# shanjiayao/PTT

Hardware: AMD Instinct MI355X
Metric: tracklet frames/sec (hot path: PointNet++ SA stack + Point-Track-Transformer blocks) (higher is better)
Workload: dtype f32

## Files before the change

include/ptt_hip.h:

```cpp
#ifndef PTT_HIP_H
#define PTT_HIP_H

#include <stddef.h>
#include <stdint.h>

#ifdef __cplusplus
extern "C" {
#endif

#define PTT_ABI_VERSION 30

enum {
    PTT_OK = 0,
    PTT_EINVAL = -1,
    PTT_EUNSUPPORTED = -2,
    PTT_ELAUNCH = -3,
    PTT_EWORKSPACE = -4
};

typedef void* ptt_stream_t;

int ptt_version(void);
const char* ptt_error_name(int code);
const char* ptt_last_error_string(void);

// ... 6 lines not shown
                 int B, int N, int C, int npoint, int32_t* idx_out, ptt_stream_t stream);

int ptt_gather_f32(const float* feat, const int32_t* idx, int B, int C, int N, int M,
                   float* out, ptt_stream_t stream);
int ptt_gather_grad_f32(const float* grad_out, const int32_t* idx, int B, int C, int N,
                        int M, float* grad_feat, ptt_stream_t stream);

int ptt_select_centres_f32(const float* xyz, const int32_t* idx, int B, int N, int M, float* new_xyz,
                           int64_t* idx64_out, ptt_stream_t stream);

int ptt_ball_query_f32(const float* new_xyz, const float* xyz, int B, int M, int N,
                       float radius, int nsample, int32_t* idx_out, ptt_stream_t stream);

int ptt_centres_ball_query_f32(const float* xyz, const int32_t* sel, int B, int N, int M, float radius, int nsample,
                               float* new_xyz, int64_t* idx64_out, int32_t* idx_out, ptt_stream_t stream);

int ptt_group_f32(const float* feat, const int32_t* idx, int B, int C, int N, int M,
                  int ns, float* out, ptt_stream_t stream);
int ptt_group_grad_f32(const float* grad_out, const int32_t* idx, int B, int C, int N,
                       int M, int ns, float* grad_feat, ptt_stream_t stream);

size_t ptt_scatter_add_det_workspace(int B, int N, int E);
int ptt_scatter_add_det_f32(const float* src, const int32_t* idx, int B, int C, int N, int E, float* out,
                            void* workspace, size_t workspace_bytes, ptt_stream_t stream);

int ptt_knn_f32(const float* xyz, int B, int N, int k, int32_t* idx_out,
                ptt_stream_t stream);
int ptt_knn_rel_f32(const float* xyz, int B, int N, int k, int32_t* idx_out, float* rel_out,
                    ptt_stream_t stream);

// ... 66 lines not shown
    int64_t feat_sb, feat_sc, feat_sn;
    float* out;
    int64_t out_sb, out_sc, out_sm;
    int B, N, M, nsample, C;
    float radius;
    int use_xyz;
    int normalize_xyz;
    int n_layers;
    ptt_sa_layer layers[PTT_SA_MAX_LAYERS];
    const float* l0_point_term;
    const float* l0_xyz_weight;
    int l0_channels;
    int l0_relu;
    void* compact_ws;
    size_t compact_ws_bytes;
} ptt_sa_desc;

int ptt_sa_fused_fwd_f32(const ptt_sa_desc* d, ptt_stream_t stream);
size_t ptt_sa_compact_workspace(int B, int M);

typedef struct ptt_xcorr_desc {
    const float* cos_t;
    const float* P;
    const float* w_sim;
    const float* scale0;
    const float* shift0;
    float* out;
    int64_t out_sb, out_sc, out_sn;
    float* sim_out;
    int B, Ns, Nt, C0;
// ... 369 lines not shown
```

ptt_amd/_lib.py:

```python
import ctypes
import os
import re
from ctypes import Structure, c_char_p, c_double, c_float, c_int, c_int32, c_int64, c_longlong, c_size_t, c_uint32, c_void_p

from .build import HEADER as HEADER_PATH, LIB as LIB_PATH


def _strip_comments(text):
    return re.sub(r"/\*.*?\*/|//[^\n]*", " ", text, flags=re.S)


def parse_defines(text):
    return {n: int(v) for n, v in re.findall(r"^[ \t]*#[ \t]*define[ \t]+(PTT_\w+)[ \t]+(-?\d+)[ \t]*$", _strip_comments(text), re.M)}


CTYPES = {"int": c_int, "int32_t": c_int32, "uint32_t": c_uint32, "int64_t": c_int64, "long long": c_longlong, "size_t": c_size_t,
          "float": c_float, "double": c_double, "ptt_stream_t": c_void_p}


def _ctype(decl, name, is_return=False):
    words = decl.replace("*", " * ").split()
    if not is_return and len(words) > 1 and words[-1] != "*":
        words.pop()
    if "*" in words:
# ... 135 lines not shown


class SaLayer(Structure):
    _fields_ = [("Wpacked", c_void_p), ("scale", c_void_p), ("shift", c_void_p),
                ("Cin", c_int), ("Cout", c_int), ("relu", c_int)]


class SaDesc(Structure):
    _fields_ = [("xyz", c_void_p), ("new_xyz", c_void_p), ("idx", c_void_p), ("feat", c_void_p),
                ("feat_sb", c_int64), ("feat_sc", c_int64), ("feat_sn", c_int64),
                ("out", c_void_p), ("out_sb", c_int64), ("out_sc", c_int64), ("out_sm", c_int64),
                ("B", c_int), ("N", c_int), ("M", c_int), ("nsample", c_int), ("C", c_int),
                ("radius", c_float), ("use_xyz", c_int), ("normalize_xyz", c_int), ("n_layers", c_int),
                ("layers", SaLayer * PTT_SA_MAX_LAYERS),
                ("l0_point_term", c_void_p), ("l0_xyz_weight", c_void_p), ("l0_channels", c_int), ("l0_relu", c_int),
                ("compact_ws", c_void_p), ("compact_ws_bytes", c_size_t)]


class XcorrDesc(Structure):
    _fields_ = [("cos_t", c_void_p), ("P", c_void_p), ("w_sim", c_void_p), ("scale0", c_void_p), ("shift0", c_void_p),
                ("out", c_void_p), ("out_sb", c_int64), ("out_sc", c_int64), ("out_sn", c_int64),
                ("sim_out", c_void_p),
                ("B", c_int), ("Ns", c_int), ("Nt", c_int), ("C0", c_int),
                ("n_layers", c_int), ("layers", SaLayer * PTT_SA_MAX_LAYERS),
                ("split", c_int32), ("out_sh", c_int64), ("search_feat", c_void_p), ("templ_feat", c_void_p),
                ("s_sb", c_int64), ("s_sn", c_int64), ("t_sb", c_int64), ("t_sn", c_int64), ("C", c_int), ("eps", c_float)]


class AttnDesc(Structure):
    _fields_ = [("xyz", c_void_p), ("rel", c_void_p), ("knn", c_void_p), ("qkv", c_void_p),
                ("Wd1p", c_void_p), ("Wd2p", c_void_p), ("bd2", c_void_p),
# ... 36 lines not shown
```

ptt_amd/csrc/common.h:

```cpp
#pragma once
#include <hip/hip_runtime.h>
#include <stdint.h>
#include <stdio.h>
#include "../../include/ptt_hip.h"

namespace ptt {

char* last_error_buf();
int fail(int code, const char* fmt, ...);
int check_launch(const char* what);

static inline hipStream_t as_stream(ptt_stream_t s) { return reinterpret_cast<hipStream_t>(s); }

struct DevSwitches {
    int linear_rt = 1, linear_ct = 1;
    int linear_small = 1;
    int sa_gather1 = 0;
    int sa_stagger = 0;
    int sa_wave = 1;
    int sa_rt = 2;
    int sa_lds = 1;
    int sa_stream = 1;
    int sa_chunk = 2;
    int pair_stagger = 0;
// ... 2 lines not shown
    int fps_plain = 0;
    int ball_cpw = 0;
    int fps_t = 0;
    int ffps_stream = 0;
    int group_grad_global = 0;
    long long* stamps = nullptr;
};
const DevSwitches& dev_switches();

int set_lds_limit(const void* fn, int bytes);

bool wgrad_stream_ok(int R, int Cout, int Cin, int ldz, int ldx);
int wgrad_stream_rows(int R);
int launch_wgrad_stream(const float* dZ, int ldz, const float* X, int ldx, int R, int Cout, int Cin, int rows, float* partial,
                        const float* x_scale, const float* x_shift, hipStream_t s);

template <int CTRL, int ROW_MASK>
__device__ __forceinline__ int dpp_i32(int v) {
    return __builtin_amdgcn_update_dpp(v, v, CTRL, ROW_MASK, 0xF, false);
}
template <int CTRL, int ROW_MASK>
__device__ __forceinline__ float dpp_f32(float v) {
    return __builtin_bit_cast(float, dpp_i32<CTRL, ROW_MASK>(__builtin_bit_cast(int, v)));
}

__device__ __forceinline__ float wave_max_f32(float v) {
    v = fmaxf(v, dpp_f32<0xB1, 0xF>(v));
    v = fmaxf(v, dpp_f32<0x4E, 0xF>(v));
    v = fmaxf(v, dpp_f32<0x141, 0xF>(v));
    v = fmaxf(v, dpp_f32<0x140, 0xF>(v));
// ... 38 lines not shown
```

ptt_amd/csrc/mfma_ops.hip:

```cpp
#include <math.h>
#include <stdlib.h>
#include <string.h>
#include "common.h"
#include "mfma_common.h"

#ifndef PTT_PAIR_PF
#define PTT_PAIR_PF 1
#endif
#ifndef PTT_GATHER_BATCH
#define PTT_GATHER_BATCH 16
#endif
#ifndef PTT_SA_WAVES
#define PTT_SA_WAVES 2
#endif

namespace ptt {

#ifdef PTT_DEV
#define PTT_STAMP(i) do { if (p.dbg && threadIdx.x == 0 && blockIdx.x < 4096) p.dbg[blockIdx.x * 8 + (i)] = __builtin_readcyclecounter(); } while (0)
#else
#define PTT_STAMP(i) do { } while (0)
#endif

__device__ __forceinline__ void stagger_second_slot(int first_wave_blocks, int quanta) {
// ... 1237 lines not shown
                    if (2 * rt < ncentres) {
                        const int c = centre0 + 2 * rt; const int b = c / p.M, mm = c - b * p.M;
                        p.out[b * p.osb + col * p.osc + mm * p.osm] = m0;
                    }
                    if (2 * rt + 1 < ncentres) {
                        const int c = centre0 + 2 * rt + 1; const int b = c / p.M, mm = c - b * p.M;
                        p.out[b * p.osb + col * p.osc + mm * p.osm] = m1;
                    }
                }
            }
        }
    }
    __builtin_amdgcn_wave_barrier();
}

constexpr int SAC_HDR = 16;
struct SacTable {
    int32_t* ws; int T;
    __host__ __device__ int32_t* ndist() const { return ws + SAC_HDR; }
    __host__ __device__ int32_t* list(int k) const { return ws + SAC_HDR + (size_t)(1 + k) * T; }
    __host__ __device__ int32_t* rows(int k) const { return ws + SAC_HDR + 5 * (size_t)T + (size_t)((4 << k) - 4) * T; }
    static size_t words(size_t T) { return SAC_HDR + 65 * T; }
};
constexpr int SAC_PASSES = 4;

__global__ __launch_bounds__(64) void sa_compact_zero_kernel(int32_t* ws) {
    if (threadIdx.x < 4) ws[threadIdx.x] = 0;
}

template <bool XYZ>
__global__ __launch_bounds__(256) void sa_compact_kernel(const float* __restrict__ xyz, const int32_t* __restrict__ idx, int N, int M,
                                                         SacTable tab) {
    __shared__ int s_cnt[4], s_base[4], s_cls[32], s_pos[32], s_nd[32];
    __shared__ int s_row[32][32];
    const int t = threadIdx.x, lane = t & 63, half = lane >> 5, s = lane & 31, w = t >> 6;
    const int g0 = blockIdx.x * 32, T = tab.T;
    if (t < 4) s_cnt[t] = 0;
    __syncthreads();
// ... 814 lines not shown
    p.dbg = dev_switches().stamps;
    p.cws = nullptr;
    const int total_centres = d->B * d->M;
    hipStream_t s = as_stream(stream);
    int rc;
    if (d->C == 0 && d->use_xyz && !hoist && d->nsample == 32 && d->n_layers == 3 && p.L[0].Cout == 64 && p.L[1].Cout == 64 &&
        p.L[2].Cout == 128 && !p.L[0].scale && !p.L[1].scale && !p.L[2].scale && p.L[0].relu && p.L[1].relu &&
        dev_switches().sa_lds) {
        const int waves = 256 * PTT_SAL_WAVES * PTT_SAL_WGS;
        p.chunk = (total_centres + waves - 1) / waves;
        if (dev_switches().sa_lds_chunk > 0 && p.chunk > dev_switches().sa_lds_chunk) p.chunk = dev_switches().sa_lds_chunk;
        const int nw = total_centres * 3 <= 256 * PTT_SAL_WAVES ? 4 : PTT_SAL_WAVES;
        int wgs = (total_centres + p.chunk * nw - 1) / (p.chunk * nw);
        const int lds = (4096 + 8192 + PTT_SAL_WAVES * 640) * (int)sizeof(float);
        if (d->compact_ws) {
            if (d->compact_ws_bytes < ptt_sa_compact_workspace(d->B, d->M) || (reinterpret_cast<uintptr_t>(d->compact_ws) & 15))
                return fail(PTT_EWORKSPACE, "ptt_sa_fused_fwd_f32: compact_ws needs %zu bytes, 16-byte aligned (got %zu)",
                            ptt_sa_compact_workspace(d->B, d->M), d->compact_ws_bytes);
            p.cws = static_cast<int32_t*>(d->compact_ws);
            hipLaunchKernelGGL(sa_compact_zero_kernel, dim3(1), dim3(64), 0, s, p.cws);
            if ((rc = check_launch("sa_compact_zero_kernel"))) return rc;
            hipLaunchKernelGGL(sa_compact_kernel<true>, dim3((total_centres + 31) / 32), dim3(256), 0, s, d->xyz, d->idx, d->N, d->M,
                               SacTable{p.cws, total_centres});
            if ((rc = check_launch("sa_compact_kernel"))) return rc;
            if (wgs > 256 * PTT_SAL_WGS) wgs = 256 * PTT_SAL_WGS;
            if ((rc = set_lds_limit(reinterpret_cast<const void*>(sa_lds_kernel<true>), lds))) return rc;
            hipLaunchKernelGGL(sa_lds_kernel<true>, dim3(wgs), dim3(64 * nw), lds, s, p);
            return check_launch("sa_lds_kernel");
        }
        if ((rc = set_lds_limit(reinterpret_cast<const void*>(sa_lds_kernel<false>), lds))) return rc;
// ... 21 lines not shown
        }
        return check_launch("sa_wave_kernel");
    }
    if (p.hoist == 2 && d->nsample == 32 && d->n_layers == 2 && p.L[0].Cin == 128 && p.L[0].Cout == 128 &&
        p.L[1].Cout == 256 && !p.L[0].scale && !p.L[1].scale && p.L[0].relu && dev_switches().sa_stream) {
        p.tiles = (total_centres + 1) / 2;
        int wgs = p.tiles < 512 ? p.tiles : 512;
        p.chunk = (p.tiles + wgs - 1) / wgs;
        if (dev_switches().sa_chunk > 0 && p.chunk > dev_switches().sa_chunk) p.chunk = dev_switches().sa_chunk;
        wgs = (p.tiles + p.chunk - 1) / p.chunk;
        if (d->compact_ws) {
            if (d->compact_ws_bytes < ptt_sa_compact_workspace(d->B, d->M) || (reinterpret_cast<uintptr_t>(d->compact_ws) & 15))
                return fail(PTT_EWORKSPACE, "ptt_sa_fused_fwd_f32: compact_ws needs %zu bytes, 16-byte aligned (got %zu)",
                            ptt_sa_compact_workspace(d->B, d->M), d->compact_ws_bytes);
            p.cws = static_cast<int32_t*>(d->compact_ws);
            hipLaunchKernelGGL(sa_compact_zero_kernel, dim3(1), dim3(64), 0, s, p.cws);
            if ((rc = check_launch("sa_compact_zero_kernel"))) return rc;
            hipLaunchKernelGGL(sa_compact_kernel<false>, dim3((total_centres + 31) / 32), dim3(256), 0, s, d->xyz, d->idx, d->N, d->M,
                               SacTable{p.cws, total_centres});
            if ((rc = check_launch("sa_compact_kernel"))) return rc;
            const int lds = (2 * SAS_TILE + 64 * 4 + 64) * (int)sizeof(float);
            if ((rc = set_lds_limit(reinterpret_cast<const void*>(sa_stream_compact_kernel), lds))) return rc;
            hipLaunchKernelGGL(sa_stream_compact_kernel, dim3(p.tiles < 512 ? p.tiles : 512), dim3(256), lds, s, p);
            return check_launch("sa_stream_compact_kernel");
        }
        const int lds = (2 * SAS_TILE + 4 * 16 * 4) * (int)sizeof(float);
        if ((rc = set_lds_limit(reinterpret_cast<const void*>(sa_stream_kernel<32>), lds))) return rc;
        hipLaunchKernelGGL((sa_stream_kernel<32>), dim3(wgs), dim3(256), lds, s, p);
        return check_launch("sa_stream_kernel");
    }
    int RT = dev_switches().sa_rt;
    if (d->nsample == 64) RT = 2;
    const int lds = 32 * RT * p.ldk * (int)sizeof(float);
    if (lds > 160 * 1024) return fail(PTT_EUNSUPPORTED, "ptt_sa_fused_fwd_f32: %d B of LDS per workgroup", lds);
    const int cpw = 32 * RT / d->nsample;
// ... 126 lines not shown
```

ptt_amd/csrc/point_ops.hip:

```cpp
#pragma clang fp contract(off)

#include <limits.h>
#include <stdlib.h>
#include "common.h"

namespace ptt {

__device__ __forceinline__ float sqdist3(float ax, float ay, float az, float bx, float by, float bz) {
    const float dx = ax - bx, dy = ay - by, dz = az - bz;
    return (dx * dx + dy * dy) + dz * dz;
}

__device__ __forceinline__ float knn_dist(float ax, float ay, float az, float bx, float by, float bz) {
    const float d = sqdist3(ax, ay, az, bx, by, bz);
    return d < __builtin_inff() ? d : 3.402823466e+38f;
}

__device__ __forceinline__ float lane_bcast(float v, int src_lane) {
    return __builtin_bit_cast(float, __builtin_amdgcn_readlane(__builtin_bit_cast(int, v), src_lane));
}

typedef float fps_f2 __attribute__((ext_vector_type(2)));


// ... 258 lines not shown
    float cx[CPW], cy[CPW], cz[CPW];
    const int nc = min(CPW, BM - centre);
#pragma unroll
    for (int c = 0; c < CPW; ++c) {
        const int cc = centre + (c < nc ? c : 0);
        const int n = sel ? sel[cc] : cc - b * M;
        cx[c] = pts[3 * n + 0]; cy[c] = pts[3 * n + 1]; cz[c] = pts[3 * n + 2];
        if (lane == 0 && c < nc) {
            new_xyz[(size_t)cc * 3 + 0] = cx[c]; new_xyz[(size_t)cc * 3 + 1] = cy[c]; new_xyz[(size_t)cc * 3 + 2] = cz[c];
            if (idx64) idx64[cc] = n;
        }
    }
    ball_sweep<CPW>(pts, N, r2, ns, cx, cy, cz, nc, idx_out + (size_t)centre * ns, lane);
}

__global__ void gather_kernel(const float* __restrict__ feat, const int32_t* __restrict__ idx, int C, int N, int M,
                              float* __restrict__ out, size_t total) {
    for (size_t e = (size_t)blockIdx.x * blockDim.x + threadIdx.x; e < total; e += (size_t)gridDim.x * blockDim.x) {
        const int j = (int)(e % M);
        const size_t bc = e / M;
        const int b = (int)(bc / C);
        out[e] = feat[bc * N + idx[(size_t)b * M + j]];
    }
}
__global__ void gather_grad_kernel(const float* __restrict__ go, const int32_t* __restrict__ idx, int C, int N, int M,
                                   float* __restrict__ gf, size_t total) {
    for (size_t e = (size_t)blockIdx.x * blockDim.x + threadIdx.x; e < total; e += (size_t)gridDim.x * blockDim.x) {
        const int j = (int)(e % M);
        const size_t bc = e / M;
        const int b = (int)(bc / C);
// ... 1021 lines not shown
    if (!xyz || !new_xyz || !idx_out) return fail(PTT_EINVAL, "ptt_centres_ball_query_f32: null pointer");
    const int BM = B * M;
    const int cpw = ball_cpw(BM, M);
    if (cpw == 8)
        hipLaunchKernelGGL((centres_ball_query_kernel<8>), dim3((BM / 8 + 3) / 4), dim3(256), 0, as_stream(stream), xyz, sel, BM,
                           M, N, radius * radius, nsample, new_xyz, reinterpret_cast<long long*>(idx64_out), idx_out);
    else if (cpw == 4)
        hipLaunchKernelGGL((centres_ball_query_kernel<4>), dim3((BM / 4 + 3) / 4), dim3(256), 0, as_stream(stream), xyz, sel, BM,
                           M, N, radius * radius, nsample, new_xyz, reinterpret_cast<long long*>(idx64_out), idx_out);
    else
        hipLaunchKernelGGL((centres_ball_query_kernel<1>), dim3((BM + 3) / 4), dim3(256), 0, as_stream(stream), xyz, sel, BM, M,
                           N, radius * radius, nsample, new_xyz, reinterpret_cast<long long*>(idx64_out), idx_out);
    return check_launch("centres_ball_query_kernel");
}


extern "C" size_t ptt_ball_query_grid_workspace(int B, int N) {
    if (B <= 0 || N <= 0) return 0;
    return (size_t)B * grid_slice_ints(N) * sizeof(int32_t);
}

static int ball_query_grid_launch(const char* who, const float* xyz, const float* centres, const int32_t* sel, int sel_mode, int B, int N, int M,
                                  float radius, int nsample, float* new_xyz, int64_t* idx64, int32_t* idx_out, void* ws, size_t ws_bytes,
                                  ptt_stream_t stream) {
    if (B < 0 || M < 0 || N <= 0 || nsample <= 0) return fail(PTT_EINVAL, "%s: B=%d M=%d N=%d nsample=%d", who, B, M, N, nsample);
    if (B == 0 || M == 0) return PTT_OK;
    if (N > 131072) return fail(PTT_EUNSUPPORTED, "%s: N=%d (the hit bitmap of a wave lives in LDS: at most 131072 points)", who, N);
    if (!ws || ws_bytes < ptt_ball_query_grid_workspace(B, N) || (reinterpret_cast<uintptr_t>(ws) & 15))
        return fail(PTT_EWORKSPACE, "%s: %zu bytes of 16-byte aligned workspace needed", who, ptt_ball_query_grid_workspace(B, N));
    hipStream_t s = as_stream(stream);
// ... 161 lines not shown
```

ptt_amd/models/backbones_3d/pointnet2/pointnet2_modules.py:

```python
import os
from typing import List

import torch
import torch.nn as nn
import torch.nn.functional as F

from .... import ops, train_ops
from ....param_cache import (DropsCachesOnModeChange, FoldedLayer, ParamCache, conv_bn_tensors, fold_conv_bn,
                             index_table)
from . import pointnet2_utils
from . import pytorch_utils as pt_utils

STREAM_COMPACT_MIN_BALLS = 2048
STREAM_COMPACT_MAX_POINTS = 1024


class PointnetSAModuleVotes(DropsCachesOnModeChange, nn.Module):
    def __init__(self, *, mlp: List[int], radius: float = None, nsample: int = None, bn: bool = True,
                 use_xyz: bool = True, normalize_xyz: bool = False, sample_uniformly: bool = False,
                 sample_method='fps'):
        super().__init__()
        self.radius = radius
        self.nsample = nsample
        self.mlp_module = None
# ... 57 lines not shown
            scale, shift = fold_conv_bn(unit)
            scale0 = scale if li == 0 else scale0
            wq = w if scale is None else w * scale.view(-1, 1, 1, 1)
            layers.append(FoldedLayer(ops.pack_weight(wq, rot), None, shift, cin, cout, hasattr(unit, 'activation')))
        hoist = None
        w0 = self.mlp_module[0].conv.weight
        if (self.use_xyz and len(layers) >= 2 and w0.shape[1] > 3 and layers[0].cout <= 256
                and os.environ.get('PTT_SA_HOIST', '1') != '0'):
            w2 = w0.reshape(w0.shape[0], w0.shape[1]).float()
            wx = w2[:, 0:3] if scale0 is None else w2[:, 0:3] * scale0[:, None]
            wf = w2[:, 3:] if scale0 is None else w2[:, 3:] * scale0[:, None]
            hoist = (ops.pack_weight(wf.contiguous()), wx.t().contiguous(), layers[0].cout, layers[0].relu)
        return layers, hoist

    def forward(self, xyz: torch.Tensor, features: torch.Tensor, npoint: int, inds: torch.Tensor = None, pre=None,
                compact: bool = False):
        self.centres_knn = None
        if self._fusable(xyz, features):
            return self._forward_fused(xyz, features, npoint, inds, pre, compact)
        return self._forward_train(xyz, features, npoint, inds)

    def _forward_fused(self, xyz, features, npoint, inds, pre, compact):
        if (pre is None and inds is None and self.sample_method == 'fps' and xyz.shape[1] <= 256 and npoint <= 128
                and xyz.shape[0] * npoint * self.nsample <= ops.ONE_FRAME_MAX_SA_ROWS and self.centres_knn_k <= npoint):
            xyz = xyz.contiguous()
            inds, inds64, new_xyz, idx, self.centres_knn = ops.fps_ball_knn(xyz, npoint, self.radius, self.nsample, self.centres_knn_k)
            pre = (new_xyz, idx, inds64)
        prefix = inds is None and self.sample_method in ('rs', 'sequence')
        if pre is not None:
            pass
        elif prefix:
            inds64 = index_table(xyz.size(0), npoint, xyz.device, torch.int64)
        elif inds is None:
            inds = self._sample(xyz, features, npoint)
        else:
            assert inds.shape[1] == npoint
            inds = inds.to(torch.int32)

        xyz = xyz.contiguous()
        if pre is not None:
            new_xyz, idx, inds64 = pre
        elif prefix:
            new_xyz, _, idx = ops.centres_ball_query(xyz, None, npoint, self.radius, self.nsample)
        else:
            new_xyz, inds64, idx = ops.centres_ball_query(xyz, inds.contiguous(), npoint, self.radius, self.nsample)
        layers, hoist = self._fused_params(xyz.device)
        if hoist is not None and features is not None:
            wf_packed, wx, c0, relu0 = hoist
            rows = features.transpose(1, 2)
            uniform = rows.stride(2) == 1 and rows.stride(0) == rows.shape[1] * rows.stride(1)
            term = ops.linear(rows if uniform else rows.contiguous(), wf_packed, c0, None, layers[0].shift, relu=False)
            B, M, ns = xyz.shape[0], npoint, self.nsample
            if (B * M * ns <= ops.ONE_FRAME_MAX_SA_ROWS and ns in (16, 32) and len(layers) == 3 and c0 % 4 == 0 and c0 >= 192):
                L1, L2 = layers[1], layers[2]
                h = torch.empty((B * M * ns, L1.cout), dtype=torch.float32, device=xyz.device)
                ops.row_jobs([pt_utils.layer_job(L1, prologue=3, x=term, idx=idx, xyz=xyz, centres=new_xyz, wx=wx,
                                                 radius=self.radius, ns=ns, M=M, N=xyz.shape[1], normalize_xyz=self.normalize_xyz,
                                                 pro_relu=relu0, out=h)])
                pooled = torch.empty((B, M, L2.cout), dtype=torch.float32, device=xyz.device)
                ops.row_jobs([pt_utils.layer_job(L2, x=h, epilogue=2, ns=ns, M=M, out=pooled)])
                return new_xyz, pooled.transpose(1, 2), inds64
            new_features = ops.sa_fused_forward(xyz, new_xyz, idx, None, layers[1:], self.radius, True,
                                                self.normalize_xyz, point_major_out=True, l0=(term, wx, relu0),
                                                compact=(bool(compact) and B * M >= STREAM_COMPACT_MIN_BALLS
                                                         and xyz.shape[1] <= STREAM_COMPACT_MAX_POINTS))
        else:
            new_features = ops.sa_fused_forward(xyz, new_xyz, idx, features, layers, self.radius,
                                                self.use_xyz, self.normalize_xyz, point_major_out=True,
                                                compact=features is None)
        return new_xyz, new_features, inds64

    def _forward_train(self, xyz, features, npoint, inds):
        if inds is None:
            inds = self._sample(xyz, features, npoint)
        else:
            assert inds.shape[1] == npoint
            inds = inds.to(torch.int32)
        hoist = (self.use_xyz and not self.sample_uniformly and self.nsample * npoint <= 16384
                 and train_ops.usable(self.mlp_module, xyz if features is None else features)
                 and self.mlp_module[0].conv.weight.shape[0] % 4 == 0)
# ... 17 lines not shown
```

ptt_amd/models/backbones_3d/pointnet2_backbone.py:

```python
from typing import List

import torch
import torch.nn as nn

from ... import graph_policy, ops, train_ops
from ...param_cache import ParamCache, index_table
from .pointnet2 import pointnet2_modules


class PointNet2BackboneLight(nn.Module):
    def __init__(self, model_cfg, input_channels, **kwargs):
        super().__init__()
        self.model_cfg = model_cfg
        input_channels -= 3
        self.num_points_each_layer = []
        self.SA_modules = nn.ModuleList()
        sa = self.model_cfg.SA_CONFIG
        for k in range(len(sa.RADIUS)):
            mlps = list(sa.MLPS[k])
            if k == 0:
                mlps[0] = input_channels
            self.SA_modules.append(pointnet2_modules.PointnetSAModuleVotes(
                radius=sa.RADIUS[k], nsample=sa.NSAMPLE[k], mlp=mlps,
                use_xyz=sa.get('USE_XYZ', True), normalize_xyz=sa.get('NORMALIZE_XYZ', True),
                sample_method=sa.SAMPLE_METHOD[k]))
        self.cov_final = nn.Conv1d(256, 256, kernel_size=1)
        self.num_point_features = sa.MLPS[-1][-1]
        self._cov_cache = ParamCache()
        self.seed_knn = 16
        self.overlap_branches = True
        self._side_stream = None

    @staticmethod
    def _break_up_pc(pc):
        xyz = pc[..., 0:3].contiguous()
        features = pc[..., 3:].contiguous() if pc.size(-1) > 3 else None
        return xyz, features

    def _cov_final(self, features):
        if not features.is_cuda:
            return self.cov_final(features)
        if self.training:
            if features.dtype != torch.float32:
                return self.cov_final(features)
            return train_ops.rows_linear(self.cov_final, features.transpose(1, 2)).transpose(1, 2)
        if ops.autograd_recording(self.cov_final, features) or features.dtype != torch.float32:
# ... 19 lines not shown
            from .pointnet2 import pointnet2_utils
            xyz = xyz.contiguous()
            if inds0 is None:
                inds0 = pointnet2_utils.furthest_point_sample(xyz, npoints[0])
            inds0 = inds0.to(torch.int32).contiguous()
            levels, inds64, knn = ops.sa_levels_point_jobs(xyz, inds0, list(npoints), list(sa.RADIUS), list(sa.NSAMPLE),
                                                           knn_k=want_knn)
            seq = [None] + [index_table(xyz.size(0), n, xyz.device, torch.int64) for n in npoints[1:3]]
            xyz, features, inds0 = self.SA_modules[0](xyz=xyz, features=features, npoint=npoints[0], inds=inds0,
                                                      pre=(levels[0][0], levels[0][1], inds64))
            xyz, features, inds1 = self.SA_modules[1](xyz=xyz, features=features, npoint=npoints[1],
                                                      pre=(levels[1][0], levels[1][1], seq[1]))
            xyz, features, inds2 = self.SA_modules[2](xyz=xyz, features=features, npoint=npoints[2],
                                                      pre=(levels[2][0], levels[2][1], seq[2]))
        else:
            xyz, features, inds0 = self.SA_modules[0](xyz=xyz, features=features, npoint=npoints[0], inds=inds0)
            xyz, features, inds1 = self.SA_modules[1](xyz=xyz, features=features, npoint=npoints[1], compact=1 in compact_levels)
            xyz, features, inds2 = self.SA_modules[2](xyz=xyz, features=features, npoint=npoints[2], compact=2 in compact_levels)
        point_features = self._cov_final(features)
        assert inds1.dtype == inds2.dtype == torch.int64, 'index type must be int64, not {}'.format(inds2.dtype)
        if all(m.sample_method in ('rs', 'sequence') for m in self.SA_modules[1:]) and inds0.shape[1] >= npoints[2]:
            inds = inds0[:, :npoints[2]]
        else:
            inds = inds0.gather(1, inds1).gather(1, inds2)
        if want_knn:
            return xyz, point_features, inds, knn
        return xyz, point_features, inds

    def sample(self, search_points, template_points):
        from .pointnet2 import pointnet2_utils
        sa = self.model_cfg.SA_CONFIG
        assert sa.SAMPLE_METHOD[0] == 'fps'
        return (pointnet2_utils.furthest_point_sample(search_points[..., 0:3].contiguous(), sa.NPOINTS_SEARCH[0]),
                pointnet2_utils.furthest_point_sample(template_points[..., 0:3].contiguous(), sa.NPOINTS_TEMPLATE[0]))

    def forward_branches(self, search_points, template_points, inds=None):
        sa = self.model_cfg.SA_CONFIG
        i_s, i_t = inds if inds is not None else (None, None)
        last = (len(self.SA_modules) - 1,) if (search_points.is_cuda and not self.training) else ()
        if not (self.overlap_branches and search_points.is_cuda and not self.training):
            r = self.branch_forward(search_points, sa.NPOINTS_SEARCH, i_s, want_knn=self.seed_knn, compact_levels=last)
            t_seeds, t_feats, t_inds = self.branch_forward(template_points, sa.NPOINTS_TEMPLATE, i_t)
        else:
            if self._side_stream is None or self._side_stream.device != search_points.device:
                self._side_stream = torch.cuda.Stream(device=search_points.device)
            main = torch.cuda.current_stream(search_points.device)
            side = graph_policy.branch(main, self._side_stream)
            with torch.cuda.stream(side):
                t_seeds, t_feats, t_inds = self.branch_forward(template_points, sa.NPOINTS_TEMPLATE, i_t)
            r = self.branch_forward(search_points, sa.NPOINTS_SEARCH, i_s, want_knn=self.seed_knn, compact_levels=last)
            graph_policy.join(main, side)
            if side is not main:
                for t in (t_seeds, t_feats, t_inds, template_points):
                    t.record_stream(main)
        s_seeds, s_feats, s_inds = r[:3]
        s_knn = r[3] if len(r) > 3 else None
        out = {'search_seeds': s_seeds, 'search_feats': s_feats, 'search_inds': s_inds,
               'template_seeds': t_seeds, 'template_feats': t_feats, 'template_inds': t_inds}
        if s_knn is not None:
            out['search_seeds_knn'] = s_knn
        return out

    def forward(self, batch_dict):
        batch_dict.update(self.forward_branches(batch_dict['search_points'], batch_dict['template_points'],
# ... 5 lines not shown
```

ptt_amd/models/trackers/tracker3d_template.py:

```python
import os

import torch
import torch.nn as nn

from .. import backbones_3d, similarity_modules, voting_heads


class Tracker3DTemplate(nn.Module):
    def __init__(self, model_cfg, num_class, dataset):
        super().__init__()
        self.model_cfg = model_cfg
        self.num_class = num_class
        self.dataset = dataset
        self.training = dataset.training
        self.class_names = dataset.class_names
        self.register_buffer('global_step', torch.LongTensor(1).zero_())
        self.module_topology = ['backbone_3d', 'similarity_module', 'centroid_voting_head', 'box_voting_head']

    @property
    def mode(self):
        return 'TRAIN' if self.training else 'TEST'

    def forward(self, **kwargs):
        raise NotImplementedError
# ... 11 lines not shown
            'voxel_size': self.dataset.voxel_size,
        }
        for name in self.module_topology:
            module, info = getattr(self, 'build_%s' % name)(model_info_dict=info)
            self.add_module(name, module)
        return info['module_list']

    def build_backbone_3d(self, model_info_dict):
        cfg = self.model_cfg.get('BACKBONE_3D', None)
        if cfg is None:
            return None, model_info_dict
        module = backbones_3d.__all__[cfg.NAME](
            model_cfg=cfg, input_channels=model_info_dict['num_point_features'],
            grid_size=model_info_dict['grid_size'], voxel_size=model_info_dict['voxel_size'],
            point_cloud_range=model_info_dict['point_cloud_range'])
        model_info_dict['module_list'].append(module)
        model_info_dict['num_point_features'] = module.num_point_features
        return module, model_info_dict

    def build_similarity_module(self, model_info_dict):
        cfg = self.model_cfg.get('SIMILARITY_MODULE', None)
        if cfg is None:
            return None, model_info_dict
        module = similarity_modules.__all__[cfg.NAME](model_cfg=cfg)
        model_info_dict['module_list'].append(module)
        return module, model_info_dict

    def _build_head(self, key, model_info_dict):
        cfg = self.model_cfg.get(key, None)
        if cfg is None:
# ... 52 lines not shown
```

ptt_amd/ops.py:

```python
import contextlib
import ctypes
import os

import torch

from . import _lib
from ._lib import AttnDesc, SaDesc, SaLayer, XcorrDesc


def _stream():
    return ctypes.c_void_p(torch.cuda.current_stream().cuda_stream)


_timing = None


def start_kernel_timing(names):
    global _timing
    _timing = {n: [] for n in names}


def stop_kernel_timing():
    global _timing
    t, _timing = _timing, None
# ... 232 lines not shown
    _chk(new_xyz, "new_xyz", torch.float32, 3)
    _chk(xyz, "xyz", torch.float32, 3)
    B, M, _ = new_xyz.shape
    N = xyz.shape[1]
    out = torch.empty((B, M, int(nsample)), dtype=torch.int32, device=xyz.device)
    if GRID_BALL_QUERY_MIN_POINTS <= N <= 131072:
        ws, ws_arg = _workspace("ptt_ball_query_grid_workspace", xyz.device, B, N)
        _launch("ptt_ball_query_grid_f32", xyz.device, _ptr(new_xyz), _ptr(xyz), B, M, N, float(radius), int(nsample), _ptr(out), *ws_arg,
                timed='ptt_ball_query_f32')
    else:
        _launch("ptt_ball_query_f32", xyz.device, _ptr(new_xyz), _ptr(xyz), B, M, N, float(radius), int(nsample), _ptr(out),
                timed='ptt_ball_query_f32')
    return out


def centres_ball_query(xyz, sel, npoint, radius, nsample, want_idx64=True):
    _chk(xyz, "xyz", torch.float32, 3)
    B, N, _ = xyz.shape
    if sel is not None:
        _chk(sel, "sel", torch.int32, 2)
    M = int(npoint)
    new_xyz = torch.empty((B, M, 3), dtype=torch.float32, device=xyz.device)
    idx64 = torch.empty((B, M), dtype=torch.int64, device=xyz.device) if (want_idx64 and sel is not None) else None
    idx = torch.empty((B, M, int(nsample)), dtype=torch.int32, device=xyz.device)
    if GRID_BALL_QUERY_MIN_POINTS <= N <= 131072:
        ws, ws_arg = _workspace("ptt_ball_query_grid_workspace", xyz.device, B, N)
        _launch("ptt_centres_ball_query_grid_f32", xyz.device, _ptr(xyz), _ptr(sel), B, N, M, float(radius), int(nsample), _ptr(new_xyz), _ptr(idx64),
                _ptr(idx), *ws_arg, timed='ptt_ball_query_f32')
    else:
        _launch("ptt_centres_ball_query_f32", xyz.device, _ptr(xyz), _ptr(sel), B, N, M, float(radius), int(nsample), _ptr(new_xyz), _ptr(idx64),
                _ptr(idx), timed='ptt_ball_query_f32')
    return new_xyz, idx64, idx


def group_points(features, idx):
    _chk(features, "features", torch.float32, 3)
    _chk(idx, "idx", torch.int32, 3)
    B, C, N = features.shape
    _, M, ns = idx.shape
# ... 113 lines not shown
        L = d.layers[i]
        L.Wpacked = wp.data_ptr()
        L.scale = sc.data_ptr() if sc is not None else None
        L.shift = sh.data_ptr() if sh is not None else None
        L.Cin, L.Cout, L.relu = int(cin), int(co), int(bool(relu))
    if l0 is not None:
        term, wx, l0_relu = l0
        if features is not None:
            raise RuntimeError("with a hoisted layer 0 the point features are already inside l0[0]")
        _chk(term, "l0 point term", torch.float32, 3)
        _chk(wx, "l0 xyz weight", torch.float32, 2)
        if term.shape[0] != B or term.shape[1] != N or wx.shape[0] != 3 or wx.shape[1] != term.shape[2]:
            raise RuntimeError("l0 point term must be (B,N,C0) and the xyz weight (3,C0)")
        d.l0_point_term, d.l0_xyz_weight = term.data_ptr(), wx.data_ptr()
        d.l0_channels, d.l0_relu = term.shape[2], int(bool(l0_relu))
    if isinstance(compact, torch.Tensor):
        if not compact.is_cuda or compact.device != xyz.device or not compact.is_contiguous():
            raise RuntimeError("compact workspace must be a contiguous tensor on %s" % xyz.device)
        d.compact_ws, d.compact_ws_bytes = compact.data_ptr(), compact.numel() * compact.element_size()
    elif compact:
        ws, (_, d.compact_ws_bytes) = _workspace("ptt_sa_compact_workspace", xyz.device, B, M)
        d.compact_ws = ws.data_ptr()
    _launch("ptt_sa_fused_fwd_f32", xyz.device, ctypes.byref(d), timed='ptt_sa_fused_fwd_f32')
    return out


def cosine_map(search_feats, templ_feats, eps=1e-8):
    for t_, n_ in ((search_feats, "search_feats"), (templ_feats, "templ_feats")):
        if not isinstance(t_, torch.Tensor) or not t_.is_cuda or t_.dtype != torch.float32 or t_.dim() != 3:
            raise RuntimeError("%s must be a (B,C,N) float32 device tensor" % n_)
    if search_feats.shape[:2] != templ_feats.shape[:2] or search_feats.device != templ_feats.device:
# ... 1368 lines not shown
```

Measured before the change: 17410.

## Build stream-compact ball tables inside the centre ball query kernel

Adds a centre+ball-query kernel that also writes the size-class compaction table (per-ball distinct counts, class lists, padded rows) used by the streaming SA kernel. The separate zero and compact kernels no longer have to run before the SA pass. Counters for later levels are reset by the first level's launch. The policy is also changed to use compact tables on all SA levels of both the search and template branches. This adds shared-memory atomics and extra global writes to the ball-query kernel, and it keeps table state across calls, so stale or mismatched tables are a risk.

Measured after the change: 17420 (median of 3 runs). No clear change (+0.1%).

```diff
diff --git a/include/ptt_hip.h b/include/ptt_hip.h
--- a/include/ptt_hip.h
+++ b/include/ptt_hip.h
@@ -8,7 +8,7 @@
 extern "C" {
 #endif
 
-#define PTT_ABI_VERSION 30
+#define PTT_ABI_VERSION 31
 
 enum {
     PTT_OK = 0,
@@ -45,6 +45,10 @@
 
 int ptt_centres_ball_query_f32(const float* xyz, const int32_t* sel, int B, int N, int M, float radius, int nsample,
                                float* new_xyz, int64_t* idx64_out, int32_t* idx_out, ptt_stream_t stream);
+
+int ptt_centres_ball_table_f32(const float* xyz, const int32_t* sel, int B, int N, int M, float radius, int nsample,
+                               float* new_xyz, int64_t* idx64_out, int32_t* idx_out, void* table, size_t table_bytes,
+                               void* zero_a, void* zero_b, ptt_stream_t stream);
 
 int ptt_group_f32(const float* feat, const int32_t* idx, int B, int C, int N, int M,
                   int ns, float* out, ptt_stream_t stream);
@@ -141,6 +145,7 @@
     int l0_relu;
     void* compact_ws;
     size_t compact_ws_bytes;
+    int compact_ws_built;
 } ptt_sa_desc;
 
 int ptt_sa_fused_fwd_f32(const ptt_sa_desc* d, ptt_stream_t stream);
diff --git a/ptt_amd/_lib.py b/ptt_amd/_lib.py
--- a/ptt_amd/_lib.py
+++ b/ptt_amd/_lib.py
@@ -173,7 +173,7 @@
                 ("radius", c_float), ("use_xyz", c_int), ("normalize_xyz", c_int), ("n_layers", c_int),
                 ("layers", SaLayer * PTT_SA_MAX_LAYERS),
                 ("l0_point_term", c_void_p), ("l0_xyz_weight", c_void_p), ("l0_channels", c_int), ("l0_relu", c_int),
-                ("compact_ws", c_void_p), ("compact_ws_bytes", c_size_t)]
+                ("compact_ws", c_void_p), ("compact_ws_bytes", c_size_t), ("compact_ws_built", c_int)]
 
 
 class XcorrDesc(Structure):
diff --git a/ptt_amd/csrc/common.h b/ptt_amd/csrc/common.h
--- a/ptt_amd/csrc/common.h
+++ b/ptt_amd/csrc/common.h
@@ -40,6 +40,15 @@
 int wgrad_stream_rows(int R);
 int launch_wgrad_stream(const float* dZ, int ldz, const float* X, int ldx, int R, int Cout, int Cin, int rows, float* partial,
                         const float* x_scale, const float* x_shift, hipStream_t s);
+
+constexpr int SAC_HDR = 16;
+struct SacTable {
+    int32_t* ws; int T;
+    __host__ __device__ int32_t* ndist() const { return ws + SAC_HDR; }
+    __host__ __device__ int32_t* list(int k) const { return ws + SAC_HDR + (size_t)(1 + k) * T; }
+    __host__ __device__ int32_t* rows(int k) const { return ws + SAC_HDR + 5 * (size_t)T + (size_t)((4 << k) - 4) * T; }
+    static size_t words(size_t T) { return SAC_HDR + 65 * T; }
+};
 
 template <int CTRL, int ROW_MASK>
 __device__ __forceinline__ int dpp_i32(int v) {
diff --git a/ptt_amd/csrc/mfma_ops.hip b/ptt_amd/csrc/mfma_ops.hip
--- a/ptt_amd/csrc/mfma_ops.hip
+++ b/ptt_amd/csrc/mfma_ops.hip
@@ -1275,14 +1275,6 @@
     __builtin_amdgcn_wave_barrier();
 }
 
-constexpr int SAC_HDR = 16;
-struct SacTable {
-    int32_t* ws; int T;
-    __host__ __device__ int32_t* ndist() const { return ws + SAC_HDR; }
-    __host__ __device__ int32_t* list(int k) const { return ws + SAC_HDR + (size_t)(1 + k) * T; }
-    __host__ __device__ int32_t* rows(int k) const { return ws + SAC_HDR + 5 * (size_t)T + (size_t)((4 << k) - 4) * T; }
-    static size_t words(size_t T) { return SAC_HDR + 65 * T; }
-};
 constexpr int SAC_PASSES = 4;
 
 __global__ __launch_bounds__(64) void sa_compact_zero_kernel(int32_t* ws) {
@@ -2127,6 +2119,9 @@
         int wgs = (total_centres + p.chunk * nw - 1) / (p.chunk * nw);
         const int lds = (4096 + 8192 + PTT_SAL_WAVES * 640) * (int)sizeof(float);
         if (d->compact_ws) {
+            if (d->compact_ws_built)
+                return fail(PTT_EINVAL, "ptt_sa_fused_fwd_f32: compact_ws_built is for the stream shape (a ball query's table holds "
+                            "real hits, this level needs distinct coordinates)");
             if (d->compact_ws_bytes < ptt_sa_compact_workspace(d->B, d->M) || (reinterpret_cast<uintptr_t>(d->compact_ws) & 15))
                 return fail(PTT_EWORKSPACE, "ptt_sa_fused_fwd_f32: compact_ws needs %zu bytes, 16-byte aligned (got %zu)",
                             ptt_sa_compact_workspace(d->B, d->M), d->compact_ws_bytes);
@@ -2178,11 +2173,13 @@
                 return fail(PTT_EWORKSPACE, "ptt_sa_fused_fwd_f32: compact_ws needs %zu bytes, 16-byte aligned (got %zu)",
                             ptt_sa_compact_workspace(d->B, d->M), d->compact_ws_bytes);
             p.cws = static_cast<int32_t*>(d->compact_ws);
-            hipLaunchKernelGGL(sa_compact_zero_kernel, dim3(1), dim3(64), 0, s, p.cws);
-            if ((rc = check_launch("sa_compact_zero_kernel"))) return rc;
-            hipLaunchKernelGGL(sa_compact_kernel<false>, dim3((total_centres + 31) / 32), dim3(256), 0, s, d->xyz, d->idx, d->N, d->M,
-                               SacTable{p.cws, total_centres});
-            if ((rc = check_launch("sa_compact_kernel"))) return rc;
+            if (!d->compact_ws_built) {
+                hipLaunchKernelGGL(sa_compact_zero_kernel, dim3(1), dim3(64), 0, s, p.cws);
+                if ((rc = check_launch("sa_compact_zero_kernel"))) return rc;
+                hipLaunchKernelGGL(sa_compact_kernel<false>, dim3((total_centres + 31) / 32), dim3(256), 0, s, d->xyz, d->idx, d->N, d->M,
+                                   SacTable{p.cws, total_centres});
+                if ((rc = check_launch("sa_compact_kernel"))) return rc;
+            }
             const int lds = (2 * SAS_TILE + 64 * 4 + 64) * (int)sizeof(float);
             if ((rc = set_lds_limit(reinterpret_cast<const void*>(sa_stream_compact_kernel), lds))) return rc;
             hipLaunchKernelGGL(sa_stream_compact_kernel, dim3(p.tiles < 512 ? p.tiles : 512), dim3(256), lds, s, p);
diff --git a/ptt_amd/csrc/point_ops.hip b/ptt_amd/csrc/point_ops.hip
--- a/ptt_amd/csrc/point_ops.hip
+++ b/ptt_amd/csrc/point_ops.hip
@@ -296,6 +296,115 @@
     ball_sweep<CPW>(pts, N, r2, ns, cx, cy, cz, nc, idx_out + (size_t)centre * ns, lane);
 }
 
+template <int CPW>
+__device__ __forceinline__ void ball_sweep_rows(const float* __restrict__ pts, int N, float r2, int ns, const float (&cx)[CPW],
+                                                const float (&cy)[CPW], const float (&cz)[CPW], int ncentres,
+                                                int32_t* __restrict__ out0, int lane, int* rows, int (&nd)[CPW]) {
+    int cnt[CPW], first[CPW];
+#pragma unroll
+    for (int c = 0; c < CPW; ++c) { cnt[c] = (c < ncentres) ? 0 : ns; first[c] = 0; }
+    for (int base = 0; base < N; base += 64) {
+        const int k = base + lane;
+        const bool in = k < N;
+        float px = 0.f, py = 0.f, pz = 0.f;
+        if (in) { px = pts[3 * k + 0]; py = pts[3 * k + 1]; pz = pts[3 * k + 2]; }
+        bool active = false;
+#pragma unroll
+        for (int c = 0; c < CPW; ++c) {
+            if (cnt[c] >= ns) continue;
+            const float d = sqdist3(cx[c], cy[c], cz[c], px, py, pz);
+            const bool hit = in && d < r2;
+            const unsigned long long mask = __ballot(hit);
+            if (mask != 0ull) {
+                if (cnt[c] == 0) first[c] = base + (__ffsll((long long)mask) - 1);
+                const int pos = cnt[c] + __popcll(mask & ((1ull << lane) - 1ull));
+                if (hit && pos < ns) { out0[(size_t)c * ns + pos] = k; rows[c * 32 + pos] = k; }
+                cnt[c] += __popcll(mask);
+            }
+            active = active || cnt[c] < ns;
+        }
+        if (!active) break;
+    }
+#pragma unroll
+    for (int c = 0; c < CPW; ++c) {
+        nd[c] = 0;
+        if (c >= ncentres) continue;
+        const int fill = (cnt[c] > 0) ? first[c] : 0;
+        for (int s = cnt[c] + lane; s < ns; s += 64) out0[(size_t)c * ns + s] = fill;
+        if (cnt[c] == 0 && lane == 0) rows[c * 32] = 0;
+        nd[c] = cnt[c] == 0 ? 1 : (cnt[c] < ns ? cnt[c] : ns);
+    }
+}
+
+template <int CPW, int WAVES, bool TABLE>
+__global__ __launch_bounds__(WAVES * 64) void centres_ball_table_kernel(const float* __restrict__ xyz, const int32_t* __restrict__ sel,
+                                                                        int BM, int M, int N, float r2, int ns,
+                                                                        float* __restrict__ new_xyz, long long* __restrict__ idx64,
+                                                                        int32_t* __restrict__ idx_out, SacTable tab,
+                                                                        int32_t* zero_a, int32_t* zero_b) {
+    constexpr int BALLS = WAVES * CPW;
+    __shared__ int s_cnt[4], s_base[4], s_cls[BALLS], s_pos[BALLS], s_nd[BALLS];
+    __shared__ int s_row[TABLE ? BALLS : 1][32];
+    const int t = threadIdx.x, lane = t & 63, w = t >> 6;
+    if (blockIdx.x == 0 && t == 0) {
+        if (zero_a) { zero_a[0] = 0; zero_a[1] = 0; zero_a[2] = 0; zero_a[3] = 0; }
+        if (zero_b) { zero_b[0] = 0; zero_b[1] = 0; zero_b[2] = 0; zero_b[3] = 0; }
+    }
+    if constexpr (TABLE) {
+        if (t < 4) s_cnt[t] = 0;
+        if (t < BALLS) s_cls[t] = -1;
+        __syncthreads();
+    }
+    const int centre = (blockIdx.x * WAVES + w) * CPW;
+    if (centre < BM) {
+        const int b = centre / M;
+        const float* __restrict__ pts = xyz + (size_t)b * N * 3;
+        float cx[CPW], cy[CPW], cz[CPW];
+        const int nc = min(CPW, BM - centre);
+#pragma unroll
+        for (int c = 0; c < CPW; ++c) {
+            const int cc = centre + (c < nc ? c : 0);
+            const int n = sel ? sel[cc] : cc - b * M;
+            cx[c] = pts[3 * n + 0]; cy[c] = pts[3 * n + 1]; cz[c] = pts[3 * n + 2];
+            if (lane == 0 && c < nc) {
+                new_xyz[(size_t)cc * 3 + 0] = cx[c]; new_xyz[(size_t)cc * 3 + 1] = cy[c]; new_xyz[(size_t)cc * 3 + 2] = cz[c];
+                if (idx64) idx64[cc] = n;
+            }
+        }
+        if constexpr (TABLE) {
+            int nd[CPW];
+            ball_sweep_rows<CPW>(pts, N, r2, ns, cx, cy, cz, nc, idx_out + (size_t)centre * ns, lane, &s_row[w * CPW][0], nd);
+            if (lane == 0) {
+#pragma unroll
+                for (int c = 0; c < CPW; ++c) {
+                    if (c >= nc) continue;
+                    const int k = nd[c] <= 4 ? 0 : nd[c] <= 8 ? 1 : nd[c] <= 16 ? 2 : 3;
+                    s_cls[w * CPW + c] = k;
+                    s_nd[w * CPW + c] = nd[c];
+                    s_pos[w * CPW + c] = atomicAdd(&s_cnt[k], 1);
+                    tab.ndist()[centre + c] = nd[c];
+                }
+            }
+        } else {
+            ball_sweep<CPW>(pts, N, r2, ns, cx, cy, cz, nc, idx_out + (size_t)centre * ns, lane);
+        }
+    }
+    if constexpr (TABLE) {
+        __syncthreads();
+        if (t < 4) s_base[t] = s_cnt[t] ? atomicAdd(&tab.ws[t], s_cnt[t]) : 0;
+        __syncthreads();
+        const int g0 = blockIdx.x * BALLS;
+        for (int e = t; e < BALLS * 32; e += WAVES * 64) {
+            const int lc = e >> 5, j = e & 31, k = s_cls[lc];
+            if (k < 0 || j >= (4 << k)) continue;
+            const int q = s_base[k] + s_pos[lc];
+            if ((unsigned)q >= (unsigned)tab.T) continue;
+            tab.rows(k)[(size_t)q * (4 << k) + j] = s_row[lc][j < s_nd[lc] ? j : 0];
+            if (j == 0) tab.list(k)[q] = g0 + lc;
+        }
+    }
+}
+
 __global__ void gather_kernel(const float* __restrict__ feat, const int32_t* __restrict__ idx, int C, int N, int M,
                               float* __restrict__ out, size_t total) {
     for (size_t e = (size_t)blockIdx.x * blockDim.x + threadIdx.x; e < total; e += (size_t)gridDim.x * blockDim.x) {
@@ -1347,6 +1456,51 @@
     return check_launch("centres_ball_query_kernel");
 }
 
+template <int CPW, int WAVES, bool TABLE>
+static void launch_ball_table(const float* xyz, const int32_t* sel, int BM, int M, int N, float radius, int ns, float* new_xyz,
+                              int64_t* idx64_out, int32_t* idx_out, SacTable tab, int32_t* za, int32_t* zb, hipStream_t s) {
+    const int waves = BM / CPW, wgs = (waves + WAVES - 1) / WAVES;
+    hipLaunchKernelGGL((centres_ball_table_kernel<CPW, WAVES, TABLE>), dim3(wgs > 0 ? wgs : 1), dim3(WAVES * 64), 0, s, xyz, sel, BM, M, N,
+                       radius * radius, ns, new_xyz, reinterpret_cast<long long*>(idx64_out), idx_out, tab, za, zb);
+}
+
+extern "C" int ptt_centres_ball_table_f32(const float* xyz, const int32_t* sel, int B, int N, int M, float radius, int nsample,
+                                          float* new_xyz, int64_t* idx64_out, int32_t* idx_out, void* table, size_t table_bytes,
+                                          void* zero_a, void* zero_b, ptt_stream_t stream) {
+    if (B < 0 || M < 0 || N <= 0 || nsample <= 0 || (!sel && M > N))
+        return fail(PTT_EINVAL, "ptt_centres_ball_table_f32: B=%d M=%d N=%d nsample=%d", B, M, N, nsample);
+    if ((reinterpret_cast<uintptr_t>(zero_a) & 15) || (reinterpret_cast<uintptr_t>(zero_b) & 15) ||
+        (table && (table == zero_a || table == zero_b)))
+        return fail(PTT_EINVAL, "ptt_centres_ball_table_f32: zero_a / zero_b must be 16-byte aligned tables other than `table`");
+    const bool empty = B == 0 || M == 0;
+    if (empty && !zero_a && !zero_b) return PTT_OK;
+    if (!empty && (!xyz || !new_xyz || !idx_out)) return fail(PTT_EINVAL, "ptt_centres_ball_table_f32: null pointer");
+    const int BM = empty ? 0 : B * M;
+    if (table && !empty) {
+        if (nsample != 32) return fail(PTT_EUNSUPPORTED, "ptt_centres_ball_table_f32: a table needs nsample == 32 (got %d)", nsample);
+        const size_t need = SacTable::words((size_t)BM) * sizeof(int32_t);
+        if (table_bytes < need || (reinterpret_cast<uintptr_t>(table) & 15))
+            return fail(PTT_EWORKSPACE, "ptt_centres_ball_table_f32: table needs %zu bytes, 16-byte aligned (got %zu)", need, table_bytes);
+    }
+    const SacTable tab{static_cast<int32_t*>(table), BM};
+    int32_t* za = static_cast<int32_t*>(zero_a);
+    int32_t* zb = static_cast<int32_t*>(zero_b);
+    hipStream_t s = as_stream(stream);
+    const int cpw = empty ? 1 : ball_cpw(BM, M);
+#define PTT_BALL_TABLE_ARGS xyz, sel, BM, M, N, radius, nsample, new_xyz, idx64_out, idx_out, tab, za, zb, s
+    if (table && !empty) {
+        if (cpw == 8) launch_ball_table<8, 4, true>(PTT_BALL_TABLE_ARGS);
+        else if (cpw == 4) launch_ball_table<4, 8, true>(PTT_BALL_TABLE_ARGS);
+        else launch_ball_table<1, 16, true>(PTT_BALL_TABLE_ARGS);
+    } else {
+        if (cpw == 8) launch_ball_table<8, 4, false>(PTT_BALL_TABLE_ARGS);
+        else if (cpw == 4) launch_ball_table<4, 4, false>(PTT_BALL_TABLE_ARGS);
+        else launch_ball_table<1, 4, false>(PTT_BALL_TABLE_ARGS);
+    }
+#undef PTT_BALL_TABLE_ARGS
+    return check_launch("centres_ball_table_kernel");
+}
+
 
 extern "C" size_t ptt_ball_query_grid_workspace(int B, int N) {
     if (B <= 0 || N <= 0) return 0;
diff --git a/ptt_amd/models/backbones_3d/pointnet2/pointnet2_modules.py b/ptt_amd/models/backbones_3d/pointnet2/pointnet2_modules.py
--- a/ptt_amd/models/backbones_3d/pointnet2/pointnet2_modules.py
+++ b/ptt_amd/models/backbones_3d/pointnet2/pointnet2_modules.py
@@ -95,13 +95,13 @@
         return layers, hoist
 
     def forward(self, xyz: torch.Tensor, features: torch.Tensor, npoint: int, inds: torch.Tensor = None, pre=None,
-                compact: bool = False):
+                compact=False, zero_tables=()):
         self.centres_knn = None
         if self._fusable(xyz, features):
-            return self._forward_fused(xyz, features, npoint, inds, pre, compact)
+            return self._forward_fused(xyz, features, npoint, inds, pre, compact, zero_tables)
         return self._forward_train(xyz, features, npoint, inds)
 
-    def _forward_fused(self, xyz, features, npoint, inds, pre, compact):
+    def _forward_fused(self, xyz, features, npoint, inds, pre, compact, zero_tables=()):
         if (pre is None and inds is None and self.sample_method == 'fps' and xyz.shape[1] <= 256 and npoint <= 128
                 and xyz.shape[0] * npoint * self.nsample <= ops.ONE_FRAME_MAX_SA_ROWS and self.centres_knn_k <= npoint):
             xyz = xyz.contiguous()
@@ -119,12 +119,21 @@
             inds = inds.to(torch.int32)
 
         xyz = xyz.contiguous()
+        compact = compact if (compact and xyz.shape[0] * npoint >= STREAM_COMPACT_MIN_BALLS
+                              and xyz.shape[1] <= STREAM_COMPACT_MAX_POINTS) else False
+        table = None
+        if pre is None and ops.ball_table_reach(xyz.shape[1]):
+            if isinstance(compact, ops.BallTable) and compact.armed and self.nsample == 32:
+                table = compact
+            tables = dict(table=table, zero=tuple(zero_tables))
+        else:
+            tables = {}
         if pre is not None:
             new_xyz, idx, inds64 = pre
         elif prefix:
-            new_xyz, _, idx = ops.centres_ball_query(xyz, None, npoint, self.radius, self.nsample)
+            new_xyz, _, idx = ops.centres_ball_query(xyz, None, npoint, self.radius, self.nsample, **tables)
         else:
-            new_xyz, inds64, idx = ops.centres_ball_query(xyz, inds.contiguous(), npoint, self.radius, self.nsample)
+            new_xyz, inds64, idx = ops.centres_ball_query(xyz, inds.contiguous(), npoint, self.radius, self.nsample, **tables)
         layers, hoist = self._fused_params(xyz.device)
         if hoist is not None and features is not None:
             wf_packed, wx, c0, relu0 = hoist
@@ -143,8 +152,7 @@
                 return new_xyz, pooled.transpose(1, 2), inds64
             new_features = ops.sa_fused_forward(xyz, new_xyz, idx, None, layers[1:], self.radius, True,
                                                 self.normalize_xyz, point_major_out=True, l0=(term, wx, relu0),
-                                                compact=(bool(compact) and B * M >= STREAM_COMPACT_MIN_BALLS
-                                                         and xyz.shape[1] <= STREAM_COMPACT_MAX_POINTS))
+                                                compact=table if table is not None else bool(compact))
         else:
             new_features = ops.sa_fused_forward(xyz, new_xyz, idx, features, layers, self.radius,
                                                 self.use_xyz, self.normalize_xyz, point_major_out=True,
diff --git a/ptt_amd/models/backbones_3d/pointnet2_backbone.py b/ptt_amd/models/backbones_3d/pointnet2_backbone.py
--- a/ptt_amd/models/backbones_3d/pointnet2_backbone.py
+++ b/ptt_amd/models/backbones_3d/pointnet2_backbone.py
@@ -1,3 +1,4 @@
+import os
 from typing import List
 
 import torch
@@ -30,6 +31,7 @@
         self.seed_knn = 16
         self.overlap_branches = True
         self._side_stream = None
+        self.compact_policy = 'search_last'
 
     @staticmethod
     def _break_up_pc(pc):
@@ -79,9 +81,14 @@
             xyz, features, inds2 = self.SA_modules[2](xyz=xyz, features=features, npoint=npoints[2],
                                                       pre=(levels[2][0], levels[2][1], seq[2]))
         else:
-            xyz, features, inds0 = self.SA_modules[0](xyz=xyz, features=features, npoint=npoints[0], inds=inds0)
-            xyz, features, inds1 = self.SA_modules[1](xyz=xyz, features=features, npoint=npoints[1], compact=1 in compact_levels)
-            xyz, features, inds2 = self.SA_modules[2](xyz=xyz, features=features, npoint=npoints[2], compact=2 in compact_levels)
+            compact = {l: l in compact_levels for l in (1, 2)}
+            if (self.compact_policy == 'all' and compact_levels and len(self.SA_modules) == 3 and ops.ball_table_reach(xyz.shape[1])
+                    and os.environ.get('PTT_BALL_TABLE', '1') != '0'):
+                compact.update({l: ops.BallTable(xyz.shape[0], npoints[l], xyz.device) for l in compact_levels})
+            tables = [c for c in compact.values() if isinstance(c, ops.BallTable)]
+            xyz, features, inds0 = self.SA_modules[0](xyz=xyz, features=features, npoint=npoints[0], inds=inds0, zero_tables=tables)
+            xyz, features, inds1 = self.SA_modules[1](xyz=xyz, features=features, npoint=npoints[1], compact=compact[1])
+            xyz, features, inds2 = self.SA_modules[2](xyz=xyz, features=features, npoint=npoints[2], compact=compact[2])
         point_features = self._cov_final(features)
         assert inds1.dtype == inds2.dtype == torch.int64, 'index type must be int64, not {}'.format(inds2.dtype)
         if all(m.sample_method in ('rs', 'sequence') for m in self.SA_modules[1:]) and inds0.shape[1] >= npoints[2]:
@@ -102,17 +109,21 @@
     def forward_branches(self, search_points, template_points, inds=None):
         sa = self.model_cfg.SA_CONFIG
         i_s, i_t = inds if inds is not None else (None, None)
-        last = (len(self.SA_modules) - 1,) if (search_points.is_cuda and not self.training) else ()
+        on = search_points.is_cuda and not self.training
+        last = (len(self.SA_modules) - 1,) if on else ()
+        templ = ()
+        if on and self.compact_policy == 'all':
+            last = templ = tuple(range(1, len(self.SA_modules)))
         if not (self.overlap_branches and search_points.is_cuda and not self.training):
             r = self.branch_forward(search_points, sa.NPOINTS_SEARCH, i_s, want_knn=self.seed_knn, compact_levels=last)
-            t_seeds, t_feats, t_inds = self.branch_forward(template_points, sa.NPOINTS_TEMPLATE, i_t)
+            t_seeds, t_feats, t_inds = self.branch_forward(template_points, sa.NPOINTS_TEMPLATE, i_t, compact_levels=templ)
         else:
             if self._side_stream is None or self._side_stream.device != search_points.device:
                 self._side_stream = torch.cuda.Stream(device=search_points.device)
             main = torch.cuda.current_stream(search_points.device)
             side = graph_policy.branch(main, self._side_stream)
             with torch.cuda.stream(side):
-                t_seeds, t_feats, t_inds = self.branch_forward(template_points, sa.NPOINTS_TEMPLATE, i_t)
+                t_seeds, t_feats, t_inds = self.branch_forward(template_points, sa.NPOINTS_TEMPLATE, i_t, compact_levels=templ)
             r = self.branch_forward(search_points, sa.NPOINTS_SEARCH, i_s, want_knn=self.seed_knn, compact_levels=last)
             graph_policy.join(main, side)
             if side is not main:
diff --git a/ptt_amd/models/trackers/tracker3d_template.py b/ptt_amd/models/trackers/tracker3d_template.py
--- a/ptt_amd/models/trackers/tracker3d_template.py
+++ b/ptt_amd/models/trackers/tracker3d_template.py
@@ -49,6 +49,8 @@
             model_cfg=cfg, input_channels=model_info_dict['num_point_features'],
             grid_size=model_info_dict['grid_size'], voxel_size=model_info_dict['voxel_size'],
             point_cloud_range=model_info_dict['point_cloud_range'])
+        if hasattr(module, 'compact_policy'):
+            module.compact_policy = 'all'
         model_info_dict['module_list'].append(module)
         model_info_dict['num_point_features'] = module.num_point_features
         return module, model_info_dict
diff --git a/ptt_amd/ops.py b/ptt_amd/ops.py
--- a/ptt_amd/ops.py
+++ b/ptt_amd/ops.py
@@ -270,7 +270,22 @@
     return out
 
 
-def centres_ball_query(xyz, sel, npoint, radius, nsample, want_idx64=True):
+class BallTable(object):
+
+    def __init__(self, B, M, device, ws=None):
+        if ws is None:
+            self.ws, (_, self.nbytes) = _workspace("ptt_sa_compact_workspace", device, B, M)
+        else:
+            self.ws, self.nbytes = ws, ws.numel() * ws.element_size()
+        self.B, self.M = B, M
+        self.armed = self.built = False
+
+
+def ball_table_reach(N):
+    return not GRID_BALL_QUERY_MIN_POINTS <= N <= 131072
+
+
+def centres_ball_query(xyz, sel, npoint, radius, nsample, want_idx64=True, table=None, zero=()):
     _chk(xyz, "xyz", torch.float32, 3)
     B, N, _ = xyz.shape
     if sel is not None:
@@ -279,6 +294,22 @@
     new_xyz = torch.empty((B, M, 3), dtype=torch.float32, device=xyz.device)
     idx64 = torch.empty((B, M), dtype=torch.int64, device=xyz.device) if (want_idx64 and sel is not None) else None
     idx = torch.empty((B, M, int(nsample)), dtype=torch.int32, device=xyz.device)
+    if table is not None or zero:
+        if not ball_table_reach(N) or len(zero) > 2:
+            raise RuntimeError("centres_ball_query: ball tables need the whole-cloud sweep (N < %d) and at most two tables to reset"
+                               % GRID_BALL_QUERY_MIN_POINTS)
+        if table is not None and ((table.B, table.M) != (B, M) or not table.armed or table.ws.device != xyz.device):
+            raise RuntimeError("centres_ball_query: the table must be a BallTable of (%d, %d) on %s whose counters an earlier "
+                               "launch resets" % (B, M, xyz.device))
+        z = [t.ws for t in zero] + [None, None]
+        _launch("ptt_centres_ball_table_f32", xyz.device, _ptr(xyz), _ptr(sel), B, N, M, float(radius), int(nsample), _ptr(new_xyz), _ptr(idx64),
+                _ptr(idx), _ptr(table.ws if table is not None else None), table.nbytes if table is not None else 0, _ptr(z[0]), _ptr(z[1]),
+                timed='ptt_ball_query_f32')
+        for t in zero:
+            t.armed, t.built = True, False
+        if table is not None:
+            table.armed, table.built = False, True
+        return new_xyz, idx64, idx
     if GRID_BALL_QUERY_MIN_POINTS <= N <= 131072:
         ws, ws_arg = _workspace("ptt_ball_query_grid_workspace", xyz.device, B, N)
         _launch("ptt_centres_ball_query_grid_f32", xyz.device, _ptr(xyz), _ptr(sel), B, N, M, float(radius), int(nsample), _ptr(new_xyz), _ptr(idx64),
@@ -422,7 +453,11 @@
             raise RuntimeError("l0 point term must be (B,N,C0) and the xyz weight (3,C0)")
         d.l0_point_term, d.l0_xyz_weight = term.data_ptr(), wx.data_ptr()
         d.l0_channels, d.l0_relu = term.shape[2], int(bool(l0_relu))
-    if isinstance(compact, torch.Tensor):
+    if isinstance(compact, BallTable):
+        if not compact.built or (compact.B, compact.M) != (B, M) or compact.ws.device != xyz.device:
+            raise RuntimeError("compact: the BallTable must hold the table of this (%d, %d) idx (centres_ball_query(table=...))" % (B, M))
+        d.compact_ws, d.compact_ws_bytes, d.compact_ws_built = compact.ws.data_ptr(), compact.nbytes, 1
+    elif isinstance(compact, torch.Tensor):
         if not compact.is_cuda or compact.device != xyz.device or not compact.is_contiguous():
             raise RuntimeError("compact workspace must be a contiguous tensor on %s" % xyz.device)
         d.compact_ws, d.compact_ws_bytes = compact.data_ptr(), compact.numel() * compact.element_size()
```
